# sevagh/Zen

Hardware: AMD Instinct MI355X
Metric: hops/sec (1024-hop HPR, 44.1 kHz mono) (higher is better)
Workload: dtype f32

## Files before the change

### zen_amd/blockrun/blockrun_kernel.hip

```cpp
#include "../csrc/common.h"
#include "../csrc/fft_dev.h"
#include "../csrc/masks.h"
#include "../csrc/median47_core.h"
#include "../csrc/median_net.h"
#include "blockrun_kernel.h"
#include "blockrun_first_pass.h"

#pragma clang fp contract(off)

namespace zen_blockrun {
namespace {

using zen_hip_impl::hard_mask_exact;
using PL = zfft::Plan<12>;
constexpr int N = PL::N, TF = PL::TF;
static_assert(N == NFFT && TF == 256 && HOP == 4 * TF, "four samples of a hop per thread");

constexpr int MID = TAPS / 2, MID_AL = 24, IMG_END = 255 * 16 + 64;
__device__ __forceinline__ int img_addr(int g) { return (g >> 4) * zm47::RSTR + (g & 15); }
constexpr int MIR_LO = 56, MIR_HI = 39;
static_assert(N - MIR_LO <= 16 * 254 - 24 && N / 2 + MIR_HI >= 16 * 128 + 39, "blocks 254 / 255 and 126 .. 128 read written columns");
constexpr int PC_WORD = 5184, PC_TAIL = 2052, EDGE_WORD = PC_WORD + PC_TAIL + 512 + 4;
static_assert((EDGE_WORD + 256) * 4 <= PL::LDS_FLOAT2 * 8, "lean layout must fit in the frame image");
constexpr int KEEP_WORD = PL::LDS_FLOAT2 * 2, CARRY_WORD = KEEP_WORD + HOP, WIN_WORD = CARRY_WORD + HOP;
constexpr size_t LDS_BYTES = (size_t)(WIN_WORD + 2 * HOP) * 4;
static_assert(LDS_BYTES <= LDS_BYTES_MAX, "three workgroups per CU");

__device__ __forceinline__ void lds_barrier()
{
	asm volatile("s_waitcnt lgkmcnt(0)\n\ts_barrier" ::: "memory");
}

struct TwGlobal32 {
	static constexpr bool PLAIN = true;
	static constexpr bool PACKED = true;
	const float2* __restrict__ p;
	__device__ __forceinline__ float2 get(int, int, int, int idx) const
	{
		return *reinterpret_cast<const float2*>(reinterpret_cast<const char*>(p) + (unsigned)(idx << 3));
	}
};

struct Spec {
	float2 S[16];
};

struct FwdInPre {
	float x[8], w[8];
	__device__ __forceinline__ float2 operator()(int, int slot) const { return make_float2(x[slot] * w[slot], 0.0f); }
};

struct FwdOut {
	Spec* r;
	int* img;
	__device__ __forceinline__ void operator()(int idx, float2 X, bool lower, int slot) const
	{
		r->S[slot] = X;
		if (lower || idx == (N >> 1)) {
			const float m = zfft::cabs_exact(X.x, X.y);
			const int key = __float_as_int(m);
			constexpr int CH = (TF / 16) * zm47::RSTR;
			const int tfl = idx - slot * TF;
			img[img_addr(tfl + MID_AL) + slot * CH] = key;
			if (slot == 0 && tfl >= 1 && tfl <= MIR_LO)
				img[img_addr(N - tfl + MID_AL)] = key;
			if (slot == 7 && tfl >= TF - MIR_HI)
				img[img_addr(N - 7 * TF - tfl + MID_AL)] = key;
		}
	}
};

struct InvIn {
	const Spec* r;
	const int* img;
	const float* pc;
	double thr;
	__device__ __forceinline__ float2 operator()(int idx, int slot) const
	{
		const int lo = slot * TF, hi = lo + TF - 1;
		int pi;
		if (hi <= N / 2)
			pi = idx;
		else if (lo > N / 2 && hi < N - MID)
			pi = N - idx;
		else
			pi = (idx > N / 2 && idx < N - MID) ? N - idx : (idx > N / 2 ? idx - (N - 512) + PC_TAIL : idx);
		const int g0 = hi <= N / 2 ? idx + 24 - slot * TF : TF + 24 - (idx - slot * TF);
		const float mag = __int_as_float(img[(g0 >> 4) * 20 + (g0 & 15) + (hi <= N / 2 ? slot : 15 - slot) * (TF / 16) * 20]);
		const float2 z = r->S[slot];
		const float m = hard_mask_exact(pc[pi], mag + FLT_EPSILON, thr);
		return make_float2(z.x * m, z.y * m);
	}
};

struct InvOut {
	float* Y;
	float* out;
	float* carry;
	float cola;
	__device__ __forceinline__ void operator()(int idx, float2 x, bool, int slot) const
	{
		const float y = x.x * cola;
		ZH_CHK(Y + idx, 1);
		Y[idx] = y;
		if (slot < 4) {
			ZH_CHK(out + idx, 1);
			out[idx] = carry[(slot & 3) * TF] + y;
		}
		else {
			carry[(slot & 3) * TF] = y;
		}
	}
};

template <bool SYM>
__device__ __forceinline__ void run_body(const RunArgs& a)
{
	extern __shared__ float2 lds[];
	int* img = reinterpret_cast<int*>(lds);
	float* Prow = reinterpret_cast<float*>(img + PC_WORD);
	const int tf = (int)threadIdx.x;
	float* keep = reinterpret_cast<float*>(img + KEEP_WORD) + tf;
	float* carry = reinterpret_cast<float*>(img + CARRY_WORD) + tf;
	float* win = reinterpret_cast<float*>(img + WIN_WORD) + tf;

	int s, f0, len;
	zen_blockrun_run(&a.part, (int)blockIdx.x, &s, &f0, &len);
	if (s >= a.n_streams || f0 + len > a.n_frames)
		return;
	const float* cur = a.in + (long long)s * a.in_stride + (long long)f0 * HOP;
	float* Yrow = a.Y + (long long)s * a.y_stream_stride + (long long)f0 * (2 * HOP);
	float* orow = a.out + (long long)s * a.out_stride + (long long)f0 * HOP;

	if (a.prev_frames > 0) {
		const int fc = a.prev_frames - 1 < a.n_frames - 1 ? a.prev_frames - 1 : a.n_frames - 1;
		if (fc >= f0 && fc < f0 + len) {
			const float* y = a.Y + (long long)s * a.y_stream_stride + (long long)(a.prev_frames - 1) * (2 * HOP) + HOP;
			float v[4];
#pragma unroll
			for (int i = 0; i < 4; ++i) {
				ZH_CHK(y + tf + i * TF, 1);
				v[i] = y[tf + i * TF];
			}
#pragma unroll
			for (int i = 0; i < 4; ++i) {
				ZH_CHK(a.carry + ((long long)s * HOP + tf + i * TF), 1);
				a.carry[(long long)s * HOP + tf + i * TF] = v[i];
			}
		}
	}
	float nx[4];
	{
		const float* pv = f0 > 0 ? cur - HOP : a.tail_prev + (long long)s * HOP;
		float p[4], w[8];
#pragma unroll
		for (int m = 0; m < 4; ++m) {
			ZH_CHK(pv + m * TF + tf, 1);
			ZH_CHK(cur + m * TF + tf, 1);
			p[m] = pv[m * TF + tf];
			nx[m] = cur[m * TF + tf];
		}
#pragma unroll
		for (int m = 0; m < 8; ++m) {
			ZH_CHK(a.window + m * TF + tf, 1);
			w[m] = a.window[m * TF + tf];
		}
#pragma unroll
		for (int m = 0; m < 4; ++m) {
			keep[m * TF] = p[m];
			carry[m * TF] = 0.0f;
		}
#pragma unroll
		for (int m = 0; m < 8; ++m)
			win[m * TF] = w[m];
	}
	if (tf == 0) {
		ZH_CHK(a.need + ((long long)s * a.n_frames + f0), 1);
		a.need[(long long)s * a.n_frames + f0] = 1u;
	}

	const int tf_run = tf;
	for (int k = 0; k < len; ++k) {
		const int f = f0 + k;
		int tf = tf_run, tw_off = 0;
		asm volatile("" : "+v"(tf));
		tf &= TF - 1;
		asm volatile("" : "+s"(tw_off));
		const float2* tw = a.tw + tw_off;
		float* keep = reinterpret_cast<float*>(img + KEEP_WORD) + tf;
		float* carry = reinterpret_cast<float*>(img + CARRY_WORD) + tf;
		float* win = reinterpret_cast<float*>(img + WIN_WORD) + tf;
		Spec r;
		{
			FwdInPre pre;
#pragma unroll
			for (int m = 0; m < 4; ++m) {
				pre.x[m] = keep[m * TF];
				pre.x[4 + m] = nx[m];
			}
#pragma unroll
			for (int m = 0; m < 8; ++m)
				pre.w[m] = win[m * TF];
#pragma unroll
			for (int m = 0; m < 4; ++m)
				keep[m * TF] = nx[m];
			if (f == a.n_frames - 1) {
				float* tail = a.tail_next + (long long)s * HOP;
#pragma unroll
				for (int m = 0; m < 4; ++m) {
					ZH_CHK(tail + m * TF + tf, 1);
					tail[m * TF + tf] = nx[m];
				}
			}
			FwdOut out;
			out.r = &r;
			out.img = img;
			{
				float p[8];
#pragma unroll
				for (int m = 0; m < 8; ++m)
					p[m] = pre.x[m] * pre.w[m];
				float2 Y0[16];
				first_pass16<true, SYM>(p, a.tw16, a.tw8, a.tw3_16, Y0);
#pragma unroll
				for (int c = 0; c < 16; ++c)
					lds[PL::pad_off(tf, c * (N / 16))] = Y0[c];
				zfft::frame_sync<TF>();
			}
			zfft::PassRunner<12, 1, false, true, false, FwdInPre, FwdOut, false, TwGlobal32>::run(tf, lds, TwGlobal32{tw}, pre, out, true);
		}
		lds_barrier();
		if (f >= a.n_frames - a.keep_mag_rows) {
			float* mag = a.mag + (((a.row0 + f) % a.ring_rows) + (long long)s * a.ring_rows) * N;
			for (int g = tf; g < N; g += TF) {
				ZH_CHK(mag + g, 1);
				mag[g] = __int_as_float(img[img_addr((g <= N / 2 ? g : N - g) + MID_AL)]);
			}
		}
		{
			const int v0 = img[img_addr(MID_AL)], v1 = img[img_addr(N - 1 + MID_AL)];
			for (int g = tf; g < MID_AL; g += TF)
				img[img_addr(g)] = v0;
			for (int g = N + MID_AL + tf; g < IMG_END; g += TF)
				img[img_addr(g)] = v1;
		}
		lds_barrier();
		{
			int(*edge)[64] = reinterpret_cast<int(*)[64]>(img + EDGE_WORD);
			const int lane = tf & 63, wave = __builtin_amdgcn_readfirstlane(tf >> 6);
			const int blk = wave < 2 ? tf : (lane < 32 ? 128 + lane : 192 + lane);
			zm47::Pieces pc;
			if (wave < 3)
				zm47::m47_sort_and_publish(img, edge, blk, lane, wave, tf == 0, blk == 255, pc);
			lds_barrier();
			if (wave < 3) {
				int o[16];
				zm47::m47_select(img, edge, blk, wave, pc, o);
				const int at = blk >= 224 ? PC_TAIL + (blk - 224) * 16 : blk * 16;
				if (blk <= 127 || blk >= 224) {
#pragma unroll
					for (int v = 0; v < 4; ++v)
						*reinterpret_cast<int4*>(&Prow[at + 4 * v]) = make_int4(o[4 * v], o[4 * v + 1], o[4 * v + 2], o[4 * v + 3]);
				}
				else if (blk == 128) {
					*reinterpret_cast<int4*>(&Prow[at]) = make_int4(o[0], o[1], o[2], o[3]);
				}
			}
		}
		lds_barrier();
		cur += HOP;
		if (k + 1 < len) {
#pragma unroll
			for (int m = 0; m < 4; ++m) {
				ZH_CHK(cur + m * TF + tf, 1);
				nx[m] = cur[m * TF + tf];
			}
		}
		{
			asm volatile("" : "+v"(tf));
			asm volatile("" : "+s"(tw_off));
			tf &= TF - 1;
			tw = a.tw + tw_off;
			carry = reinterpret_cast<float*>(img + CARRY_WORD) + tf;
			InvIn in;
			in.r = &r;
			in.img = img;
			in.pc = Prow;
			in.thr = a.thr;
			InvOut out;
			out.Y = Yrow;
			out.out = orow;
			out.carry = carry;
			out.cola = a.cola;
			zfft::PassRunner<12, 0, true, false, true, InvIn, InvOut, true, TwGlobal32>::run(tf, lds, TwGlobal32{tw}, in, out, true);
		}
		Yrow += 2 * HOP;
		orow += HOP;
	}
}

__global__ __launch_bounds__(256, 3) void blockrun_kernel(RunArgs a) { run_body<true>(a); }
__global__ __launch_bounds__(256, 3) void blockrun_kernel_plain_table(RunArgs a) { run_body<false>(a); }

__global__ __launch_bounds__(256) void blockrun_fixup_kernel(RunArgs a)
{
	const long long total = (long long)a.n_streams * a.n_frames;
	const long long item = (long long)blockIdx.x * 4 + (threadIdx.x >> 6);
	const int lane = threadIdx.x & 63;
	if (item >= total)
		return;
	ZH_CHK(a.need + item, 1);
	if (!a.need[item])
		return;
	const int s = (int)(item / a.n_frames), f = (int)(item - (long long)s * a.n_frames);
	const float* Y = a.Y + (long long)s * a.y_stream_stride + (long long)f * (2 * HOP);
	const float* prev = f == 0 ? a.carry + (long long)s * HOP : Y - HOP;
	float* o = a.out + (long long)s * a.out_stride + (long long)f * HOP;
	if (((reinterpret_cast<uintptr_t>(o) | reinterpret_cast<uintptr_t>(prev) | reinterpret_cast<uintptr_t>(Y)) & 15) == 0) {
		float4 p[HOP / 256], y[HOP / 256];
#pragma unroll
		for (int i = 0; i < HOP / 256; ++i) {
			const int k = i * 256 + lane * 4;
			ZH_CHK(prev + k, 4);
			ZH_CHK(Y + k, 4);
			p[i] = *reinterpret_cast<const float4*>(prev + k);
			y[i] = *reinterpret_cast<const float4*>(Y + k);
		}
#pragma unroll
		for (int i = 0; i < HOP / 256; ++i) {
			const int k = i * 256 + lane * 4;
			ZH_CHK(o + k, 4);
			*reinterpret_cast<float4*>(o + k) = make_float4(p[i].x + y[i].x, p[i].y + y[i].y, p[i].z + y[i].z, p[i].w + y[i].w);
		}
	}
	else {
		for (int k = lane; k < HOP; k += 64) {
			ZH_CHK(o + k, 1);
			ZH_CHK(prev + k, 1);
			ZH_CHK(Y + k, 1);
			o[k] = prev[k] + Y[k];
		}
	}
	if (lane == 0)
		a.need[item] = 0u;
}

}

size_t run_kernel_lds_bytes() { return LDS_BYTES; }

int launch_run(const RunArgs& a, hipStream_t stream)
{
	const long long runs = (long long)a.n_streams * a.part.runs_per_stream;
	if (a.tw_symmetric)
		hipLaunchKernelGGL(blockrun_kernel, dim3((unsigned)runs), dim3(TF), LDS_BYTES, stream, a);
	else
		hipLaunchKernelGGL(blockrun_kernel_plain_table, dim3((unsigned)runs), dim3(TF), LDS_BYTES, stream, a);
	ZH_HIP(hipGetLastError());
	return ZEN_HIP_OK;
}

int launch_fixup(const RunArgs& a, hipStream_t stream)
{
	const long long total = (long long)a.n_streams * a.n_frames;
	hipLaunchKernelGGL(blockrun_fixup_kernel, dim3((unsigned)((total + 3) / 4)), dim3(256), 0, stream, a);
	ZH_HIP(hipGetLastError());
	return ZEN_HIP_OK;
}

}
```

Measured before the change: 59.56 million.

## Replace edge-block median sorting with wave-ballot threshold counting for mask bits

The third wave no longer runs the full 47-tap median sort/select for the edge blocks (Nyquist and tail columns). Instead it computes, per output, a threshold key from the magnitude and uses wave ballots plus popcounts to decide whether the median reaches that threshold, writing a 0/1 mask value directly. The inverse-FFT input then uses this precomputed value as the mask for those edge bins. This cuts sort work and select work for wave 2, and the Nyquist magnitude write moves to a separate slot-8 path. The cost is subtle exactness logic around thresholds and infinities.

```diff
diff --git a/zen_amd/blockrun/blockrun_edge_count.h b/zen_amd/blockrun/blockrun_edge_count.h
--- /dev/null
+++ b/zen_amd/blockrun/blockrun_edge_count.h
@@ -0,0 +1,89 @@
+#pragma once
+#include <hip/hip_runtime.h>
+
+#include <cfloat>
+#include <cmath>
+#include <cstring>
+
+#pragma clang fp contract(off)
+
+namespace zen_blockrun {
+
+constexpr int EDGE_OUTPUTS = 24;
+constexpr int EDGE_KEY_INF = 0x7f800000;
+constexpr int EDGE_KEY_NONE = 0x7fffffff;
+constexpr int EDGE_IMG_COL0 = 24, EDGE_IMG_RSTR = 20;
+constexpr unsigned long long EDGE_LANES_A = (2ull << 46) - 2;
+constexpr unsigned long long EDGE_LANES_B = (2ull << 23) - 2;
+
+__device__ __forceinline__ int edge_img_addr(int col)
+{
+	const int g = col + EDGE_IMG_COL0;
+	return (g >> 4) * EDGE_IMG_RSTR + (g & 15);
+}
+
+__device__ __forceinline__ int edge_bits_of(float f)
+{
+	int i;
+	memcpy(&i, &f, sizeof(i));
+	return i;
+}
+__device__ __forceinline__ float edge_float_of(int i)
+{
+	float f;
+	memcpy(&f, &i, sizeof(f));
+	return f;
+}
+
+__device__ __forceinline__ int edge_threshold_key(double thr, int mag_key)
+{
+	const float d = edge_float_of(mag_key) + FLT_EPSILON;
+	const double t = thr * (double)d;
+	const float r = (float)t;
+	const int kr = edge_bits_of(r);
+	const int k = (double)r > t ? kr : (int)((unsigned)kr + 1u);
+	return t < (double)INFINITY ? k : EDGE_KEY_NONE;
+}
+
+__device__ __forceinline__ bool edge_count_reaches(unsigned long long m, int j)
+{
+	if (j == 0)
+		return __builtin_popcountll(m & EDGE_LANES_B) >= 12;
+	const unsigned long long lanes = (2ull << (j + 23)) - 2;
+	return __builtin_popcountll(m & lanes) + (24 - j) * (int)((m >> 1) & 1) >= 24;
+}
+
+template <class Wave>
+__device__ __forceinline__ unsigned edge_count_bits(const Wave& w)
+{
+	unsigned bits = 0;
+#pragma unroll
+	for (int j = 0; j < EDGE_OUTPUTS; ++j)
+		bits |= (unsigned)edge_count_reaches(w.ge(j == 0, w.threshold(j)), j) << j;
+	const unsigned long long na = w.ge(false, EDGE_KEY_INF + 1), nb = w.ge(true, EDGE_KEY_INF + 1);
+	if (((na & EDGE_LANES_A) | (nb & EDGE_LANES_B)) != 0) {
+#pragma unroll
+		for (int j = 0; j < EDGE_OUTPUTS; ++j)
+			bits &= ~((unsigned)edge_count_reaches(j == 0 ? nb : na, j) << j);
+	}
+	return bits;
+}
+
+#if defined(__HIPCC__)
+struct EdgeWave {
+	int a, b, k;
+	__device__ __forceinline__ unsigned long long ge(bool from_b, int K) const { return __builtin_amdgcn_ballot_w64((from_b ? b : a) >= K); }
+	__device__ __forceinline__ int threshold(int j) const { return __builtin_amdgcn_readlane(k, j); }
+};
+
+__device__ __forceinline__ unsigned edge_count_wave(const int* img, int lane, double thr, int n_half)
+{
+	EdgeWave w;
+	w.a = img[edge_img_addr(lane)];
+	w.b = img[edge_img_addr(n_half - lane)];
+	w.k = edge_threshold_key(thr, lane == 0 ? w.b : w.a);
+	return edge_count_bits(w);
+}
+#endif
+
+}
diff --git a/zen_amd/blockrun/blockrun_kernel.hip b/zen_amd/blockrun/blockrun_kernel.hip
--- a/zen_amd/blockrun/blockrun_kernel.hip
+++ b/zen_amd/blockrun/blockrun_kernel.hip
@@ -5,6 +5,7 @@
 #include "../csrc/median_net.h"
 #include "blockrun_kernel.h"
 #include "blockrun_first_pass.h"
+#include "blockrun_edge_count.h"
 
 #pragma clang fp contract(off)
 
@@ -20,6 +21,7 @@
 __device__ __forceinline__ int img_addr(int g) { return (g >> 4) * zm47::RSTR + (g & 15); }
 constexpr int MIR_LO = 56, MIR_HI = 39;
 static_assert(N - MIR_LO <= 16 * 254 - 24 && N / 2 + MIR_HI >= 16 * 128 + 39, "blocks 254 / 255 and 126 .. 128 read written columns");
+static_assert(EDGE_IMG_COL0 == MID_AL && EDGE_IMG_RSTR == zm47::RSTR && EDGE_OUTPUTS == MID + 1, "blockrun_edge_count.h reads this image");
 constexpr int PC_WORD = 5184, PC_TAIL = 2052, EDGE_WORD = PC_WORD + PC_TAIL + 512 + 4;
 static_assert((EDGE_WORD + 256) * 4 <= PL::LDS_FLOAT2 * 8, "lean layout must fit in the frame image");
 constexpr int KEEP_WORD = PL::LDS_FLOAT2 * 2, CARRY_WORD = KEEP_WORD + HOP, WIN_WORD = CARRY_WORD + HOP;
@@ -56,7 +58,11 @@
 	__device__ __forceinline__ void operator()(int idx, float2 X, bool lower, int slot) const
 	{
 		r->S[slot] = X;
-		if (lower || idx == (N >> 1)) {
+		if (slot == 8) {
+			if (__builtin_amdgcn_readfirstlane(idx) < (N >> 1) + 64 && idx == (N >> 1))
+				img[img_addr((N >> 1) + MID_AL)] = __float_as_int(zfft::cabs_exact(X.x, X.y));
+		}
+		else if (lower) {
 			const float m = zfft::cabs_exact(X.x, X.y);
 			const int key = __float_as_int(m);
 			constexpr int CH = (TF / 16) * zm47::RSTR;
@@ -88,7 +94,10 @@
 		const int g0 = hi <= N / 2 ? idx + 24 - slot * TF : TF + 24 - (idx - slot * TF);
 		const float mag = __int_as_float(img[(g0 >> 4) * 20 + (g0 & 15) + (hi <= N / 2 ? slot : 15 - slot) * (TF / 16) * 20]);
 		const float2 z = r->S[slot];
-		const float m = hard_mask_exact(pc[pi], mag + FLT_EPSILON, thr);
+		const float p = pc[pi];
+		float m = hard_mask_exact(p, mag + FLT_EPSILON, thr);
+		if (hi > N / 2 && !(lo > N / 2 && hi < N - MID))
+			m = (idx == N / 2 || idx >= N - MID) ? p : m;
 		return make_float2(z.x * m, z.y * m);
 	}
 };
@@ -248,23 +257,22 @@
 		{
 			int(*edge)[64] = reinterpret_cast<int(*)[64]>(img + EDGE_WORD);
 			const int lane = tf & 63, wave = __builtin_amdgcn_readfirstlane(tf >> 6);
-			const int blk = wave < 2 ? tf : (lane < 32 ? 128 + lane : 192 + lane);
 			zm47::Pieces pc;
-			if (wave < 3)
-				zm47::m47_sort_and_publish(img, edge, blk, lane, wave, tf == 0, blk == 255, pc);
+			if (wave < 3) {
+				zm47::m47_sort_and_publish(img, edge, tf, lane, wave, tf == 0, false, pc);
+			}
+			else {
+				const unsigned bits = edge_count_wave(img, lane, a.thr, N / 2);
+				if (lane < EDGE_OUTPUTS)
+					Prow[lane == 0 ? N / 2 : PC_TAIL + 512 - lane] = (bits >> lane) & 1u ? 1.0f : 0.0f;
+			}
 			lds_barrier();
-			if (wave < 3) {
+			if (wave < 2) {
 				int o[16];
-				zm47::m47_select(img, edge, blk, wave, pc, o);
-				const int at = blk >= 224 ? PC_TAIL + (blk - 224) * 16 : blk * 16;
-				if (blk <= 127 || blk >= 224) {
-#pragma unroll
-					for (int v = 0; v < 4; ++v)
-						*reinterpret_cast<int4*>(&Prow[at + 4 * v]) = make_int4(o[4 * v], o[4 * v + 1], o[4 * v + 2], o[4 * v + 3]);
-				}
-				else if (blk == 128) {
-					*reinterpret_cast<int4*>(&Prow[at]) = make_int4(o[0], o[1], o[2], o[3]);
-				}
+				zm47::m47_select(img, edge, tf, wave, pc, o);
+#pragma unroll
+				for (int v = 0; v < 4; ++v)
+					*reinterpret_cast<int4*>(&Prow[tf * 16 + 4 * v]) = make_int4(o[4 * v], o[4 * v + 1], o[4 * v + 2], o[4 * v + 3]);
 			}
 		}
 		lds_barrier();
```

After: 62.43 million, median of 6. +4.8%, better.
